# itshawi/data-accelerator

Hardware: AMD Instinct MI355X
Metric: events/sec (node) + p99 latency, SimulatedData IoT Flow (higher is better)
Workload: dtype fp64/int64 columns (no reduced precision)

## Files before the change

dxa/io/kafka_device.py:

```python
from __future__ import annotations

import ctypes
from dataclasses import dataclass
from typing import List, Optional, Sequence, Tuple

import numpy as np
import torch

_PLAN_ERRS = {-2: "message format is not v2", -3: "CRC mismatch", -5: "codec decoded on the host only",
              -7: "malformed compressed payload (LZ4 / snappy / zstd)", -8: "dependent-block LZ4 frame", -9: "offset deltas with gaps"}


TORCH_DT = {np.dtype(np.int32): torch.int32, np.dtype(np.int64): torch.int64, np.dtype(np.uint8): torch.uint8}


class Unsupported(Exception):
    """The fetch needs the host decoder."""


_BOUND = False


def _lib():
    global _BOUND
    from ..ops.serialize import lib
    L = lib()
    if not _BOUND:
        p, i64, i32 = ctypes.c_void_p, ctypes.c_int64, ctypes.c_int
        L.dxa_kafka_plan.argtypes = [p, i64, i64, i32, p, p] + [p] * 14
        L.dxa_kafka_plan.restype = ctypes.c_int
        _BOUND = True
    return L


@dataclass
class FetchPlan:
    b_count: np.ndarray
    b_base: np.ndarray
    b_skip: np.ndarray
    b_keep: np.ndarray
    b_first: np.ndarray
    b_nblk: np.ndarray
    b_rec0: np.ndarray
    k_comp_off: np.ndarray
    k_comp_len: np.ndarray
    k_stored: np.ndarray
    k_out_off: np.ndarray
    k_cap: np.ndarray
    out_bytes: int
    next_offset: int
    nbytes: int = 0
    packed: Optional[torch.Tensor] = None
    layout: Optional[list] = None
    b_crc_off: Optional[np.ndarray] = None
    b_crc_len: Optional[np.ndarray] = None
    b_crc: Optional[np.ndarray] = None

    def __post_init__(self):
        n = int(self.b_count.shape[0])
        for name, dt in (("b_crc_off", np.int64), ("b_crc_len", np.int32), ("b_crc", np.int32)):
            if getattr(self, name) is None:
                setattr(self, name, np.zeros(n, dt))

    @property
    def nbat(self) -> int:
        return int(self.b_count.shape[0])

    @property
    def nblk(self) -> int:
        return int(self.k_comp_off.shape[0])

    @property
    def nrec(self) -> int:
        return int(self.b_keep.sum()) if self.nbat else 0

    def last_offsets(self) -> np.ndarray:
        return self.b_base + self.b_skip + self.b_keep - 1


def plan_fetch(data, min_offset: int, verify_crc: bool = True) -> FetchPlan:
    a = np.frombuffer(data, dtype=np.uint8) if not isinstance(data, np.ndarray) else data
    L = _lib()
    counts = np.zeros(5, dtype=np.int64)
    nxt = ctypes.c_int64(0)
    rc = L.dxa_kafka_plan(a.ctypes.data, a.size, min_offset, int(verify_crc), counts.ctypes.data,
                          ctypes.byref(nxt), *([None] * 14))
    if rc:
        raise Unsupported(_PLAN_ERRS.get(rc, f"plan error {rc}"))
    nbat, nblk = int(counts[0]), int(counts[1])
    arr = dict(b_count=np.zeros(nbat, np.int32), b_base=np.zeros(nbat, np.int64),
               b_skip=np.zeros(nbat, np.int32), b_first=np.zeros(nbat, np.int32), b_nblk=np.zeros(nbat, np.int32),
               b_rec0=np.zeros(nbat, np.int64), k_comp_off=np.zeros(nblk, np.int64),
               k_comp_len=np.zeros(nblk, np.int32), k_stored=np.zeros(nblk, np.uint8),
               k_out_off=np.zeros(nblk, np.int64), k_cap=np.zeros(nblk, np.int64),
               b_crc_off=np.zeros(nbat, np.int64), b_crc_len=np.zeros(nbat, np.int32), b_crc=np.zeros(nbat, np.int32))
    order = ["b_count", "b_base", "b_skip", "b_first", "b_nblk", "b_rec0", "k_comp_off", "k_comp_len", "k_stored",
             "k_out_off", "k_cap", "b_crc_off", "b_crc_len", "b_crc"]
    rc = L.dxa_kafka_plan(a.ctypes.data, a.size, min_offset, int(verify_crc), counts.ctypes.data,
                          ctypes.byref(nxt), *[arr[k].ctypes.data for k in order])
    if rc:
        raise Unsupported(_PLAN_ERRS.get(rc, f"plan error {rc}"))
    keep = (arr["b_count"] - arr["b_skip"]).astype(np.int32)
    return FetchPlan(b_keep=keep, out_bytes=int(counts[3]), next_offset=nxt.value, nbytes=int(a.size), **arr)


_ARRAYS = [("b_count", np.int32, "b"), ("b_base", np.int64, "b"), ("b_skip", np.int32, "b"),
           ("b_keep", np.int32, "b"), ("b_first", np.int32, "b"), ("b_nblk", np.int32, "b"),
           ("b_rec0", np.int64, "b"), ("k_comp_off", np.int64, "k"), ("k_comp_len", np.int32, "k"),
           ("k_stored", np.uint8, "k"), ("k_out_off", np.int64, "k"), ("k_cap", np.int64, "k"),
           ("b_crc_off", np.int64, "b"), ("b_crc_len", np.int32, "b"), ("b_crc", np.int32, "b")]


class PlanBuffer:

    def __init__(self):
        self.buf: Optional[torch.Tensor] = None
        self.busy = None
        self.reserved = False

    def free(self) -> bool:
        return not self.reserved and (self.busy is None or self.busy.query())

    def release(self, event=None):
        self.busy = event
        self.reserved = False

    def carve(self, nbat: int, nblk: int):
        layout, pos = [], 0
        for name, dt, kind in _ARRAYS:
            cnt = nbat if kind == "b" else nblk
            layout.append((name, pos, cnt))
            pos += (cnt * np.dtype(dt).itemsize + 15) // 16 * 16
        if self.buf is None or self.buf.numel() < pos:
            self.buf = torch.empty(max(pos, 1) * 5 // 4 + 64, dtype=torch.uint8, pin_memory=torch.cuda.is_available())
        raw = self.buf.numpy()
        arrs = {name: raw[off:off + cnt * np.dtype(dt).itemsize].view(dt)
                for (name, off, cnt), (_, dt, _k) in zip(layout, _ARRAYS)}
        return arrs, layout, pos


class PlanBufferPool:

    def __init__(self):
        self.bufs: List[PlanBuffer] = []
        self._lock = __import__("threading").Lock()

    def get(self) -> PlanBuffer:
        with self._lock:
            for b in self.bufs:
                if b.free():
                    b.reserved = True
                    return b
            b = PlanBuffer()
            b.reserved = True
            self.bufs.append(b)
            return b


def plan_many(data: np.ndarray, bounds: Sequence[Tuple[int, int]], min_offsets: Sequence[int],
              threads: int = 16, buffer: Optional[PlanBuffer] = None, verify_crc: bool = True) -> FetchPlan:
    L = _lib()
    if not hasattr(L, "_plan_many_bound"):
        p, i64, i32 = ctypes.c_void_p, ctypes.c_int64, ctypes.c_int
        L.dxa_kafka_plan_count.argtypes = [p, i64, p, p, p, i32, i32, p, p]
        L.dxa_kafka_plan_fill.argtypes = [p, i64, p, p, p, i32, p] + [p] * 14
        L._plan_many_bound = True
    ns = len(bounds)
    so = np.array([b[0] for b in bounds], np.int64)
    sl = np.array([b[1] - b[0] for b in bounds], np.int64)
    mo = np.array(list(min_offsets), np.int64)
    counts = np.zeros((ns, 4), np.int64)
    nxt = np.zeros(ns, np.int64)
    rc = L.dxa_kafka_plan_count(data.ctypes.data, ns, so.ctypes.data, sl.ctypes.data, mo.ctypes.data,
                                int(verify_crc), threads,
                                counts.ctypes.data, nxt.ctypes.data)
    if rc:
        raise Unsupported(_PLAN_ERRS.get(rc, f"plan error {rc}"))
    nbat, nblk = int(counts[:, 0].sum()), int(counts[:, 1].sum())
    buffer = buffer or PlanBuffer()
    arrs, layout, used = buffer.carve(nbat, nblk)
    rc = L.dxa_kafka_plan_fill(data.ctypes.data, ns, so.ctypes.data, sl.ctypes.data, mo.ctypes.data, threads,
                               counts.ctypes.data, *[arrs[n].ctypes.data for n in
                                                     ("b_count", "b_base", "b_skip", "b_first", "b_nblk", "b_rec0",
                                                      "k_comp_off", "k_comp_len", "k_stored", "k_out_off",
                                                      "k_cap", "b_crc_off", "b_crc_len", "b_crc")])
    if rc:
        raise Unsupported(_PLAN_ERRS.get(rc, f"plan error {rc}"))
    np.subtract(arrs["b_count"], arrs["b_skip"], out=arrs["b_keep"])
    plan = FetchPlan(out_bytes=int(counts[:, 3].sum()), next_offset=int(nxt.max()) if ns else 0,
                     nbytes=int((so + sl).max()) if ns else 0, packed=buffer.buf[:used], layout=layout, **arrs)
    plan.buffer = buffer
    return plan


def merge(plans: Sequence[Tuple[FetchPlan, int]]) -> FetchPlan:
    if not plans:
        return FetchPlan(*(np.zeros(0, t) for t in (np.int32, np.int64, np.int32, np.int32, np.int32, np.int32,
                                                      np.int64, np.int64, np.int32, np.uint8, np.int64, np.int64)),
                         out_bytes=0, next_offset=0)
    cat = lambda k: np.concatenate([getattr(p, k) for p, _ in plans])
    blk0, out0, rec0 = [], [], []
    nb = ob = nr = 0
    for p, _ in plans:
        blk0.append(nb)
        out0.append(ob)
        rec0.append(nr)
        nb += p.nblk
        ob += p.out_bytes
        nr += p.nrec
    return FetchPlan(
        b_count=cat("b_count"), b_base=cat("b_base"), b_skip=cat("b_skip"), b_keep=cat("b_keep"),
        b_first=np.concatenate([p.b_first + b for (p, _), b in zip(plans, blk0)]).astype(np.int32),
        b_nblk=cat("b_nblk"),
        b_rec0=np.concatenate([_rec0(p) + r for (p, _), r in zip(plans, rec0)]),
        k_comp_off=np.concatenate([p.k_comp_off + at for p, at in plans]),
        k_comp_len=cat("k_comp_len"), k_stored=cat("k_stored"),
        k_out_off=np.concatenate([p.k_out_off + o for (p, _), o in zip(plans, out0)]),
        k_cap=cat("k_cap"), out_bytes=ob, next_offset=plans[-1][0].next_offset,
        nbytes=max(at + p.nbytes for p, at in plans),
        b_crc_off=np.concatenate([p.b_crc_off + at for p, at in plans]), b_crc_len=cat("b_crc_len"),
        b_crc=cat("b_crc"))


def _rec0(p: FetchPlan) -> np.ndarray:
    if not p.nbat:
        return np.zeros(0, np.int64)
    c = np.cumsum(p.b_keep, dtype=np.int64)
    return c - p.b_keep


def trim(p: FetchPlan, max_records: int) -> FetchPlan:
    if p.nrec <= max_records:
        return p
    keep = p.b_keep.copy()
    cum = np.cumsum(keep, dtype=np.int64)
    cut = int(np.searchsorted(cum, max_records, side="left"))
    before = int(cum[cut - 1]) if cut else 0
    keep[cut] = max_records - before
    keep[cut + 1:] = 0
    q = FetchPlan(**{**p.__dict__, "b_keep": keep.astype(np.int32)})
    q.b_rec0 = _rec0(q)
    q.next_offset = int(p.b_base[cut] + p.b_skip[cut] + keep[cut])
    return q


class DeviceRecordDecoder:

    def __init__(self, device, chunks: int = 4, copy_stream=None, decode_stream=None, track: bool = True,
                 verify_crc: bool = False):
        self.device = torch.device(device)
        self.verify_crc = verify_crc
        self.crc_stream = torch.cuda.Stream(self.device) if verify_crc else None
        self.chunks = max(1, chunks)
        cus = torch.cuda.get_device_properties(self.device).multi_processor_count
        self.min_blocks_per_chunk = cus * 64
        self.copy_stream = copy_stream or torch.cuda.Stream(self.device)
        self.decode_stream = decode_stream or torch.cuda.Stream(self.device)
        self.track = track
        self.checks: List["DecodeStatus"] = []

    def decode(self, staging: torch.Tensor, plan: FetchPlan):
        from ..engine.processor import RawBatch
        from ..ops import native as N
        dev = self.device
        n = plan.nrec
        if plan.packed is None:
            if not hasattr(self, "_packs"):
                self._packs = PlanBufferPool()
            pb = self._packs.get()
            plan.buffer = pb
            arrs, layout, used = pb.carve(plan.nbat, plan.nblk)
            for name, _dt, _k in _ARRAYS:
                arrs[name][...] = getattr(plan, name)
            packed = pb.buf[:used]
        else:
            packed, layout = plan.packed, plan.layout
        with torch.cuda.stream(self.copy_stream):
            dtab = packed.to(dev, non_blocking=True)
            ddata = torch.empty(plan.nbytes + 32, dtype=torch.uint8, device=dev)
            tab_ev = torch.cuda.Event()
            tab_ev.record(self.copy_stream)
        if getattr(plan, "buffer", None) is not None:
            plan.buffer.release(tab_ev)
        views = {name: dtab[off:off + cnt * np.dtype(dt).itemsize].view(TORCH_DT[np.dtype(dt)])
                 for (name, off, cnt), (_, dt, _k) in zip(layout, _ARRAYS)}
        tabs = [views[k] for k in ("k_comp_off", "k_comp_len", "k_stored", "k_out_off", "k_cap", "b_count",
                                   "b_skip", "b_keep", "b_first", "b_nblk", "b_rec0")]
        crc_tabs = [views[k] for k in ("b_crc_off", "b_crc_len", "b_crc")]
        co, cl, sd, oo, cap, bc, bs, bk, bf, bn, br = tabs
        with torch.cuda.stream(self.decode_stream):
            out = torch.empty(plan.out_bytes + 64, dtype=torch.uint8, device=dev)
            produced = torch.empty(max(1, plan.nblk), dtype=torch.int64, device=dev)
            bstat = torch.empty(max(1, plan.nblk), dtype=torch.int32, device=dev)
            offs = torch.empty(n + 1, dtype=torch.int64, device=dev)
            ends = torch.empty(max(1, n), dtype=torch.int64, device=dev)
            rstat = torch.empty(max(1, plan.nbat), dtype=torch.int32, device=dev)
        self.decode_stream.wait_event(tab_ev)
        st = self.decode_stream.cuda_stream
        nb = plan.nblk
        chunks = max(1, min(self.chunks, nb // max(1, self.min_blocks_per_chunk)))
        kinds = set(np.unique(plan.k_stored[:nb]).tolist()) if nb else set()
        has_gzip, has_snappy, has_zstd = 2 in kinds, 3 in kinds, 4 in kinds
        bounds = np.linspace(0, nb, chunks + 1).astype(np.int64)
        ev_last = tab_ev
        copied = 0
        for k in range(chunks):
            b0, b1 = int(bounds[k]), int(bounds[k + 1])
            if b1 <= b0:
                continue
            lo = copied
            hi = plan.nbytes if b1 == nb else int(plan.k_comp_off[b1])
            copied = hi
            N.call("dxa_memcpy_h2d_async", ddata.data_ptr() + lo, staging.data_ptr() + lo, hi - lo,
                   self.copy_stream.cuda_stream)
            ev = torch.cuda.Event()
            ev.record(self.copy_stream)
            ev_last = ev
            self.decode_stream.wait_event(ev)
            N.call("dxa_lz4_decode_into", N.ptr(ddata), N.ptr(co[b0:b1]), N.ptr(cl[b0:b1]), N.ptr(sd[b0:b1]),
                   N.ptr(oo[b0:b1]), N.ptr(cap[b0:b1]), b1 - b0, N.ptr(out), N.ptr(produced[b0:b1]),
                   N.ptr(bstat[b0:b1]), st)
            for present, entry in ((has_gzip, "dxa_inflate_into"), (has_snappy, "dxa_snappy_decode_into"),
                                   (has_zstd, "dxa_zstd_decode_into")):
                if present:
                    N.call(entry, N.ptr(ddata), N.ptr(co[b0:b1]), N.ptr(cl[b0:b1]), N.ptr(sd[b0:b1]),
                           N.ptr(oo[b0:b1]), N.ptr(cap[b0:b1]), b1 - b0, N.ptr(out), N.ptr(produced[b0:b1]),
                           N.ptr(bstat[b0:b1]), st)
        with torch.cuda.stream(self.decode_stream):
            offs[n:].fill_(plan.out_bytes)
        N.call("dxa_kafka_records", N.ptr(out), plan.nbat, N.ptr(bc), N.ptr(bs), N.ptr(bk), N.ptr(bf), N.ptr(bn),
               N.ptr(br), N.ptr(oo), N.ptr(cap), N.ptr(produced), N.ptr(bstat), N.ptr(offs), N.ptr(ends),
               N.ptr(rstat), st)
        done = torch.cuda.Event()
        done.record(self.decode_stream)
        if self.verify_crc:
            cs = self.crc_stream
            cs.wait_event(ev_last)
            with torch.cuda.stream(cs):
                cstat = torch.empty(max(1, plan.nbat), dtype=torch.int32, device=dev)
            N.call("dxa_kafka_crc", N.ptr(ddata), plan.nbat, *[N.ptr(t) for t in crc_tabs], N.ptr(cstat),
                   cs.cuda_stream)
            cs.wait_event(done)
            with torch.cuda.stream(cs):
                bad = (rstat[:plan.nbat] != 0).sum() + (cstat[:plan.nbat] != 0).sum()
                status = DecodeStatus(bad, cs)
            for t in (ddata, dtab, rstat):
                t.record_stream(cs)
        else:
            with torch.cuda.stream(self.decode_stream):
                status = DecodeStatus((rstat[:plan.nbat] != 0).sum(), self.decode_stream)
        for t in (ddata, produced, bstat, dtab):
            t.record_stream(self.decode_stream)
        if self.track:
            self.checks.append(status)
        self._inflight = [(e, b) for e, b in getattr(self, "_inflight", []) if not e.query()] + \
            [(status.event if self.verify_crc else done, (staging, packed))]
        return RawBatch(out, offs, n, ends=ends[:n], source_bytes=plan.nbytes, status=status), done

    def check(self):
        pending, self.checks = self.checks, []
        bad = sum(s.failed() for s in pending)
        if bad:
            raise DecodeError(f"{bad} Kafka record batch(es) failed to decode on the device")


class DecodeError(ValueError):
    pass


class DecodeStatus:

    __slots__ = ("host", "event")

    def __init__(self, bad: torch.Tensor, stream):
        self.host = torch.empty(1, dtype=torch.int64, pin_memory=True)
        self.host.copy_(bad.reshape(1), non_blocking=True)
        self.event = torch.cuda.Event()
        self.event.record(stream)

    def failed(self) -> int:
        self.event.synchronize()
        return int(self.host[0])

    def raise_if_failed(self, what: str = "batch"):
        bad = self.failed()
        if bad:
            raise DecodeError(f"{what}: {bad} Kafka record batch(es) failed to decode on the device")


_CRC_POLY = 0x82F63B78


def _multmodp(a: int, b: int) -> int:
    p = 0
    m = 1 << 31
    while m:
        if a & m:
            p ^= b
        b = (b >> 1) ^ _CRC_POLY if b & 1 else b >> 1
        m >>= 1
    return p


def _x2n_table():
    t, p = [], 1 << 30
    for _ in range(32):
        t.append(p)
        p = _multmodp(p, p)
    return t


_X2N = _x2n_table()


def _raw_crc(reg: int, data: bytes) -> int:
    for byte in data:
        reg ^= byte
        for _ in range(8):
            reg = (reg >> 1) ^ _CRC_POLY if reg & 1 else reg >> 1
    return reg


def _x8n(n: int) -> int:
    p, sq = 1 << 31, 1 << 30
    for _ in range(3):
        sq = _multmodp(sq, sq)
    while n:
        if n & 1:
            p = _multmodp(sq, p)
        sq = _multmodp(sq, sq)
        n >>= 1
    return p


def crc32c_segmented(data: bytes, base_align: int = 0) -> int:
    n = len(data)
    e = base_align + n
    E = e - (e & 7)
    if E - base_align < 8:
        return ~_raw_crc(0xFFFFFFFF, data) & 0xFFFFFFFF
    nrow = (E - base_align + 511) // 512
    r0 = E - nrow * 512
    msg = bytearray(data)
    for q in range(min(4, n)):
        msg[q] ^= 0xFF

    def byte_at(pos):
        q = pos - base_align
        return msg[q] if 0 <= q < n else 0
    total = 0
    for lane in range(64):
        acc = 0
        for r in range(nrow):
            a = r0 + r * 512 + lane * 8
            acc = _raw_crc(acc, bytes(byte_at(a + k) for k in range(8)))
            if r + 1 < nrow:
                acc = _multmodp(_x8n(504), acc)
        if acc:
            total ^= _multmodp(_x8n((63 - lane) * 8), acc)
    reg = _raw_crc(total, bytes(msg[E - base_align:]))
    return ~reg & 0xFFFFFFFF


def decode_on_host_like(staging: np.ndarray, plan: FetchPlan, verify_crc: bool = False):
    from ..ops import lz4
    out = np.zeros(plan.out_bytes + 64, dtype=np.uint8)
    starts, ends = [], []
    for i in range(plan.nbat):
        if verify_crc:
            lo = int(plan.b_crc_off[i])
            got = crc32c_segmented(staging[lo:lo + int(plan.b_crc_len[i])].tobytes(), lo & 7)
            if got != int(plan.b_crc[i]) & 0xFFFFFFFF:
                raise DecodeError(f"batch {i}: CRC-32C mismatch")
        f, nb = int(plan.b_first[i]), int(plan.b_nblk[i])
        p = int(plan.k_out_off[f])
        end = p
        for b in range(f, f + nb):
            src = staging[plan.k_comp_off[b]: plan.k_comp_off[b] + plan.k_comp_len[b]]
            kind = int(plan.k_stored[b])
            if kind == 2:
                import zlib
                raw = zlib.decompressobj(-15).decompress(src.tobytes())
            elif kind == 3:
                from .kafka import snappy_decompress
                raw = snappy_decompress(src.tobytes())
            elif kind == 4:
                from .kafka import zstd_decompress
                raw = zstd_decompress(src.tobytes())
            else:
                raw = src.tobytes() if kind else lz4.decompress_block(src.tobytes(), int(plan.k_cap[b]))
            out[end:end + len(raw)] = np.frombuffer(raw, np.uint8)
            end += len(raw)
        data = out

        def varint(p):
            u, s = 0, 0
            while True:
                c = int(data[p])
                p += 1
                u |= (c & 0x7F) << s
                s += 7
                if not c & 0x80:
                    return (u >> 1) ^ -(u & 1), p
        skip, keep, count = int(plan.b_skip[i]), int(plan.b_keep[i]), int(plan.b_count[i])
        for r in range(min(count, skip + keep)):
            ln, p = varint(p)
            rec_end = p + ln
            p += 1
            _, p = varint(p)
            _, p = varint(p)
            kl, p = varint(p)
            p += max(kl, 0)
            vl, p = varint(p)
            if r >= skip:
                starts.append(p)
                ends.append(p + max(vl, 0))
            p = rec_end
        assert p <= end
    return out, np.array(starts, np.int64), np.array(ends, np.int64)
```

dxa/ops/csrc/lz4.hip:

```cpp
#include "dxa_common.h"

namespace {

struct InWin {
  const uint8_t* base;
  uintptr_t wb;
  uint4 w;
  __device__ __forceinline__ uint32_t at(int64_t q) {
    const uintptr_t a = reinterpret_cast<uintptr_t>(base + q);
    const uintptr_t b = a & ~(uintptr_t)15;
    if (b != wb) {
      wb = b;
      w = *reinterpret_cast<const uint4*>(b);
    }
    return dxa::window_byte(w, (uint32_t)(a - b));
  }
};

struct OutBuf {
  uint8_t* p;
  int64_t len;
  int head;
  int nacc;
  uint64_t a0, a1;
  uintptr_t wb;
  uint4 w;

  __device__ __forceinline__ void init(uint8_t* dst) {
    p = dst; len = 0; nacc = 0; a0 = a1 = 0; wb = 0;
    head = (int)((16 - ((uintptr_t)dst & 15)) & 15);
  }
  __device__ __forceinline__ void put(uint32_t c) {
    if (len < head) {
      p[len] = (uint8_t)c;
      wb = 0;
    } else {
      if (nacc < 8) a0 |= (uint64_t)c << (8 * nacc);
      else a1 |= (uint64_t)c << (8 * (nacc - 8));
      if (++nacc == 16) {
        uint64_t* q = reinterpret_cast<uint64_t*>(p + len - 15);
        __builtin_nontemporal_store(a0, q);
        __builtin_nontemporal_store(a1, q + 1);
        a0 = a1 = 0;
        nacc = 0;
      }
    }
    ++len;
  }
  __device__ __forceinline__ uint32_t get(int64_t q) {
    const int64_t acc0 = len - nacc;
    if (q >= acc0 && len >= head) {
      const int k = (int)(q - acc0);
      return (uint32_t)(((k < 8) ? (a0 >> (8 * k)) : (a1 >> (8 * (k - 8)))) & 0xff);
    }
    const uintptr_t a = reinterpret_cast<uintptr_t>(p + q);
    const uintptr_t b = a & ~(uintptr_t)15;
    if (b != wb) {
      wb = b;
      asm volatile("" ::: "memory");
      w = *reinterpret_cast<const uint4*>(b);
    }
    return dxa::window_byte(w, (uint32_t)(a - b));
  }
  __device__ __forceinline__ void finish() {
    uint8_t* q = p + len - nacc;
    for (int k = 0; k < nacc; ++k) q[k] = (uint8_t)((k < 8 ? a0 >> (8 * k) : a1 >> (8 * (k - 8))) & 0xff);
  }
};

enum : int32_t { LZ_OK = 0, LZ_TRUNC = 1, LZ_OFFSET = 2, LZ_OVERFLOW = 3, LZ_SIZE = 4 };

template <bool WRITE>
__device__ int32_t run_block(const uint8_t* src, int64_t n, uint8_t* dst, int64_t cap, int64_t& produced) {
  InWin in{src, 0, make_uint4(0, 0, 0, 0)};
  OutBuf out;
  if (WRITE) out.init(dst);
  int64_t ip = 0, op = 0;
  while (ip < n) {
    const uint32_t token = in.at(ip++);
    int64_t lit = token >> 4;
    if (lit == 15) {
      uint32_t b;
      do { if (ip >= n) return LZ_TRUNC; b = in.at(ip++); lit += b; } while (b == 255);
    }
    if (lit > n - ip) return LZ_TRUNC;
    if (lit > cap - op) return LZ_OVERFLOW;
    if (WRITE) for (int64_t k = 0; k < lit; ++k) out.put(in.at(ip + k));
    ip += lit;
    op += lit;
    if (ip >= n) break;
    if (n - ip < 2) return LZ_TRUNC;
    const int64_t off = (int64_t)in.at(ip) | ((int64_t)in.at(ip + 1) << 8);
    ip += 2;
    if (off == 0 || off > op) return LZ_OFFSET;
    int64_t ml = token & 15;
    if (ml == 15) {
      uint32_t b;
      do { if (ip >= n) return LZ_TRUNC; b = in.at(ip++); ml += b; } while (b == 255);
    }
    ml += 4;
    if (ml > cap - op) return LZ_OVERFLOW;
    if (WRITE) {
      const int64_t s = op - off;
      if (off == 1) {
        const uint32_t c = out.get(s);
        for (int64_t k = 0; k < ml; ++k) out.put(c);
      } else {
        for (int64_t k = 0; k < ml; ++k) out.put(out.get(s + k));
      }
    }
    op += ml;
  }
  if (WRITE) out.finish();
  produced = op;
  return LZ_OK;
}

__global__ __launch_bounds__(256) void lz4_sizes_kernel(const uint8_t* __restrict__ src,
                                                        const int64_t* __restrict__ comp_off,
                                                        const int32_t* __restrict__ comp_len,
                                                        const uint8_t* __restrict__ stored, int64_t nb,
                                                        int64_t max_block, int64_t* __restrict__ out_len,
                                                        int32_t* __restrict__ status) {
  const int64_t b = (int64_t)blockIdx.x * blockDim.x + threadIdx.x;
  if (b >= nb) return;
  if (stored[b]) { out_len[b] = comp_len[b]; status[b] = LZ_OK; return; }
  int64_t produced = 0;
  const int32_t rc = run_block<false>(src + comp_off[b], comp_len[b], nullptr, max_block, produced);
  out_len[b] = rc == LZ_OK ? produced : 0;
  status[b] = rc;
}

constexpr int kWaitVm0 = 0xF70;

template <int G>
__global__ __launch_bounds__(256) void lz4_decode_group_kernel(const uint8_t* __restrict__ src,
                                                               const int64_t* __restrict__ comp_off,
                                                               const int32_t* __restrict__ comp_len,
                                                               const uint8_t* __restrict__ stored,
                                                               const int64_t* __restrict__ out_off,
                                                               const int64_t* __restrict__ out_len, int64_t nb,
                                                               uint8_t* __restrict__ dst,
                                                               int32_t* __restrict__ status,
                                                               int64_t* __restrict__ produced) {
  static_assert(G == 8 || G == 16, "group width");
  constexpr int NW = 16 / G, LPL = 16 / G, BPL = 32 / G, LOG_G = G == 8 ? 3 : 4;
  constexpr int WB = 64, PIPE = 32;
  const int64_t b = ((int64_t)blockIdx.x * 256 + threadIdx.x) / G;
  const int gl = (int)(threadIdx.x & (G - 1));
  const int gbase = (int)((threadIdx.x & 63) & ~(G - 1));
  if (b >= nb) return;
  const uint8_t kd = stored[b];
  if (kd > 1) return;
  const int32_t n = comp_len[b];
  const int64_t cap64 = out_len[b];
  const uint8_t* in = src + comp_off[b];
  uint8_t* out = dst + out_off[b];
  auto put = [&](bool on, int32_t pos, uint32_t v) {
    if (on) out[pos] = (uint8_t)v;
  };
  auto fetch = [&](bool on, int32_t pos) -> uint32_t { return on ? (uint32_t)out[pos] : 0u; };
  if (kd) {
    if (produced ? (n > cap64) : (n != cap64)) {
      if (gl == 0) status[b] = LZ_SIZE;
      return;
    }
    for (int32_t k = gl; k < n; k += G) out[k] = in[k];
    if (gl == 0) {
      status[b] = LZ_OK;
      if (produced) produced[b] = n;
    }
    return;
  }
  if (cap64 > INT32_MAX || cap64 < 0 || n < 0) {
    if (gl == 0) status[b] = LZ_OVERFLOW;
    return;
  }
  const int32_t cap = (int32_t)cap64;
  const int32_t shift = (int32_t)(reinterpret_cast<uintptr_t>(in) & 3);
  const uint8_t* a0 = in - shift;
  const int32_t lim = shift + n + 16;
  uint32_t X[NW];
  auto ld = [&](int32_t w0) {
#pragma unroll
    for (int k = 0; k < NW; ++k) {
      const int32_t q = w0 + 4 * (gl + G * k);
      X[k] = (q + 4 <= lim) ? *reinterpret_cast<const uint32_t*>(a0 + q) : 0u;
    }
    __builtin_amdgcn_s_waitcnt(kWaitVm0);
  };
  auto wbyte = [&](int32_t r) -> uint32_t {
    const int d = (r >> 2) & (G * NW - 1);
    const int addr = (gbase + (d & (G - 1))) << 2;
    uint32_t v = (uint32_t)__builtin_amdgcn_ds_bpermute(addr, (int)X[0]);
    if constexpr (NW == 2) {
      const uint32_t v1 = (uint32_t)__builtin_amdgcn_ds_bpermute(addr, (int)X[1]);
      v = (d >> LOG_G) ? v1 : v;
    }
    return (v >> ((r & 3) * 8)) & 0xffu;
  };
  int32_t xb = 0;
  ld(0);
  auto get = [&](int32_t p) -> uint32_t {
    if (p - xb >= WB) {
      xb = p & ~3;
      ld(xb);
    }
    return wbyte(p - xb);
  };
  const int32_t iend = shift + n;
  int32_t ip = shift, op = 0, rc = LZ_OK, done = 0;
  int32_t pdst = 0, pml = 0;
  uint32_t pv[BPL];
#pragma unroll
  for (int k = 0; k < BPL; ++k) pv[k] = 0;
  auto flush = [&]() {
#pragma unroll
    for (int k = 0; k < BPL; ++k) put(gl + G * k < pml, pdst + G * k + gl, pv[k]);
  };
  while (ip < iend) {
    if (ip - xb > WB - 16) {
      xb = ip & ~3;
      ld(xb);
    }
    const int32_t r = ip - xb;
    const uint32_t token = wbyte(r);
    int32_t lit = (int32_t)(token >> 4);
    const int32_t mlc = (int32_t)(token & 15);
    const bool has_ext = mlc == 15 && lit < 15 && r + lit + 4 <= WB;
    const uint32_t mext = has_ext ? wbyte(r + lit + 3) : 0u;
    const int32_t fml = mlc + 4 + (int32_t)mext;
    const int32_t fhdr = lit + 3 + (mlc == 15 ? 1 : 0);
    if (lit < 15 && (mlc < 15 || mext < 255) && r + fhdr <= WB && iend - ip >= fhdr && cap - op >= lit + fml) {
#pragma unroll
      for (int k = 0; k < LPL; ++k) {
        const uint32_t lv = wbyte(r + 1 + G * k + gl);
        put(gl + G * k < lit, op + G * k + gl, lv);
      }
      const int32_t off = (int32_t)(wbyte(r + 1 + lit) | (wbyte(r + 2 + lit) << 8));
      ip += fhdr;
      op += lit;
      if (off == 0 || off > op) { rc = LZ_OFFSET; break; }
      const int32_t ml = fml;
      const int32_t s0 = op - off;
      const int32_t src_end = s0 + (off < ml ? off : ml);
      if (pml > 0 && (src_end > pdst || ml > PIPE)) {
        flush();
        pml = 0;
      }
      if (src_end > done) {
        __builtin_amdgcn_s_waitcnt(kWaitVm0);
        asm volatile("" ::: "memory");
        done = pml > 0 ? pdst : op;
      }
      if (ml > PIPE) {
        if (off >= ml) {
          for (int32_t c = 0; c < ml; c += G)
            if (c + gl < ml) out[op + c + gl] = out[s0 + c + gl];
        } else {
          for (int32_t c = 0; c < ml; c += G) {
            const uint32_t i = (uint32_t)(c + gl);
            if ((int32_t)i < ml) out[op + i] = out[s0 + (int32_t)(i % (uint32_t)off)];
          }
        }
        op += ml;
        continue;
      }
      uint32_t v[BPL];
      if (off >= ml) {
#pragma unroll
        for (int k = 0; k < BPL; ++k) v[k] = fetch(gl + G * k < ml, s0 + G * k + gl);
      } else {
        const uint32_t o = (uint32_t)off;
#pragma unroll
        for (int k = 0; k < BPL; ++k) v[k] = fetch(gl + G * k < ml, s0 + (int32_t)((uint32_t)(gl + G * k) % o));
      }
      if (pml > 0) flush();
      pdst = op;
      pml = ml;
#pragma unroll
      for (int k = 0; k < BPL; ++k) pv[k] = v[k];
      op += ml;
      continue;
    }
    if (pml > 0) {
      flush();
      pml = 0;
    }
    ++ip;
    if (lit == 15) {
      uint32_t e;
      do {
        if (ip >= iend) { rc = LZ_TRUNC; break; }
        e = get(ip);
        ++ip;
        lit += (int32_t)e;
      } while (e == 255);
      if (rc != LZ_OK) break;
    }
    if (lit > iend - ip) { rc = LZ_TRUNC; break; }
    if (lit > cap - op) { rc = LZ_OVERFLOW; break; }
    for (int32_t c = 0; c < lit; c += G)
      if (c + gl < lit) out[op + c + gl] = a0[ip + c + gl];
    ip += lit;
    op += lit;
    if (ip >= iend) break;
    if (iend - ip < 2) { rc = LZ_TRUNC; break; }
    const int32_t off = (int32_t)(get(ip) | (get(ip + 1) << 8));
    ip += 2;
    if (off == 0 || off > op) { rc = LZ_OFFSET; break; }
    int32_t ml = mlc;
    if (ml == 15) {
      uint32_t e;
      do {
        if (ip >= iend) { rc = LZ_TRUNC; break; }
        e = get(ip);
        ++ip;
        ml += (int32_t)e;
      } while (e == 255);
      if (rc != LZ_OK) break;
    }
    ml += 4;
    if (ml > cap - op) { rc = LZ_OVERFLOW; break; }
    const int32_t s0 = op - off;
    if (s0 + (off < ml ? off : ml) > done) {
      __builtin_amdgcn_s_waitcnt(kWaitVm0);
      asm volatile("" ::: "memory");
      done = op;
    }
    if (off >= ml) {
      for (int32_t c = 0; c < ml; c += G)
        if (c + gl < ml) out[op + c + gl] = out[s0 + c + gl];
    } else {
      for (int32_t c = 0; c < ml; c += G) {
        const uint32_t i = (uint32_t)(c + gl);
        if ((int32_t)i < ml) out[op + i] = out[s0 + (int32_t)(i % (uint32_t)off)];
      }
    }
    op += ml;
  }
  if (pml > 0) flush();
  if (rc == LZ_OK && !produced && op != cap) rc = LZ_SIZE;
  if (gl == 0) {
    status[b] = rc;
    if (produced) produced[b] = op;
  }
}

}

DXA_API int dxa_lz4_block_sizes(const void* src, const void* comp_off, const void* comp_len, const void* stored,
                                int64_t nb, int64_t max_block, void* out_len, void* status, void* st) {
  if (nb <= 0) return 0;
  hipLaunchKernelGGL(lz4_sizes_kernel, dim3((unsigned)((nb + 255) / 256)), dim3(256), 0, (hipStream_t)st,
                     (const uint8_t*)src, (const int64_t*)comp_off, (const int32_t*)comp_len, (const uint8_t*)stored,
                     nb, max_block, (int64_t*)out_len, (int32_t*)status);
  return (int)hipGetLastError();
}

template <int G>
static int launch_group(int64_t nb, hipStream_t s, const uint8_t* src, const int64_t* co, const int32_t* cl,
                        const uint8_t* sd, const int64_t* oo, const int64_t* ol, uint8_t* dst, int32_t* status,
                        int64_t* produced) {
  const dim3 grid((unsigned)((nb * G + 255) / 256));
  hipLaunchKernelGGL((lz4_decode_group_kernel<G>), grid, dim3(256), 0, s, src, co, cl, sd, oo, ol, nb, dst, status,
                     produced);
  return (int)hipGetLastError();
}

DXA_API int dxa_lz4_decode(const void* src, const void* comp_off, const void* comp_len, const void* stored,
                           const void* out_off, const void* out_len, int64_t nb, int64_t max_out, void* dst,
                           void* status, void* st) {
  if (nb <= 0) return 0;
  const hipStream_t s = (hipStream_t)st;
  return launch_group<16>(nb, s, (const uint8_t*)src, (const int64_t*)comp_off, (const int32_t*)comp_len,
                          (const uint8_t*)stored, (const int64_t*)out_off, (const int64_t*)out_len, (uint8_t*)dst,
                          (int32_t*)status, (int64_t*)nullptr);
}

DXA_API int dxa_lz4_decode_into(const void* src, const void* comp_off, const void* comp_len, const void* stored,
                                const void* out_off, const void* cap, int64_t nb, void* dst, void* produced,
                                void* status, void* st) {
  if (nb <= 0) return 0;
  const hipStream_t s = (hipStream_t)st;
  const uint8_t* s8 = (const uint8_t*)src;
  const int64_t* co = (const int64_t*)comp_off;
  const int32_t* cl = (const int32_t*)comp_len;
  const uint8_t* sd = (const uint8_t*)stored;
  const int64_t* oo = (const int64_t*)out_off;
  const int64_t* cp = (const int64_t*)cap;
  return launch_group<16>(nb, s, s8, co, cl, sd, oo, cp, (uint8_t*)dst, (int32_t*)status, (int64_t*)produced);
}

DXA_API int dxa_memcpy_h2d_async(void* dst, const void* src, int64_t n, void* st) {
  if (n <= 0) return 0;
  return (int)hipMemcpyAsync(dst, src, (size_t)n, hipMemcpyHostToDevice, (hipStream_t)st);
}
```

Before: 252.2 million.

## Decode up to sixteen LZ4 sequences per lane group in parallel

Reworks the LZ4 group decoder so each 16-lane group speculatively parses sequence headers inside a 128-byte input window. It chains token positions through bpermute, prefix-sums output offsets with DPP, and copies literals and matches for many short sequences at once using wide unaligned stores. The goal is to remove the serial one-sequence-at-a-time loop that dominates small-record decoding. It also pins waves per EU, drops the G template, and lowers the minimum blocks per chunk so batches get split into more chunks. The cost is much more complex dependency handling between overlapping matches, with risk of correctness bugs and extra register pressure.

```diff
diff --git a/dxa/io/kafka_device.py b/dxa/io/kafka_device.py
--- a/dxa/io/kafka_device.py
+++ b/dxa/io/kafka_device.py
@@ -253,7 +253,7 @@
         self.crc_stream = torch.cuda.Stream(self.device) if verify_crc else None
         self.chunks = max(1, chunks)
         cus = torch.cuda.get_device_properties(self.device).multi_processor_count
-        self.min_blocks_per_chunk = cus * 64
+        self.min_blocks_per_chunk = cus * 16
         self.copy_stream = copy_stream or torch.cuda.Stream(self.device)
         self.decode_stream = decode_stream or torch.cuda.Stream(self.device)
         self.track = track
diff --git a/dxa/ops/csrc/lz4.hip b/dxa/ops/csrc/lz4.hip
--- a/dxa/ops/csrc/lz4.hip
+++ b/dxa/ops/csrc/lz4.hip
@@ -132,20 +132,23 @@
 }
 
 constexpr int kWaitVm0 = 0xF70;
-
-template <int G>
-__global__ __launch_bounds__(256) void lz4_decode_group_kernel(const uint8_t* __restrict__ src,
-                                                               const int64_t* __restrict__ comp_off,
-                                                               const int32_t* __restrict__ comp_len,
-                                                               const uint8_t* __restrict__ stored,
-                                                               const int64_t* __restrict__ out_off,
-                                                               const int64_t* __restrict__ out_len, int64_t nb,
-                                                               uint8_t* __restrict__ dst,
-                                                               int32_t* __restrict__ status,
-                                                               int64_t* __restrict__ produced) {
-  static_assert(G == 8 || G == 16, "group width");
-  constexpr int NW = 16 / G, LPL = 16 / G, BPL = 32 / G, LOG_G = G == 8 ? 3 : 4;
-  constexpr int WB = 64, PIPE = 32;
+typedef uint32_t __attribute__((aligned(1), may_alias)) u32_unaligned;
+struct __attribute__((packed, may_alias)) U8 { uint32_t a, b; };
+struct __attribute__((packed, may_alias)) U16 { uint32_t a, b, c, d; };
+
+__device__ __forceinline__ int32_t row_scan16(int32_t x) {
+  x += __builtin_amdgcn_update_dpp(0, x, 0x111, 0xf, 0xf, false);
+  x += __builtin_amdgcn_update_dpp(0, x, 0x112, 0xf, 0xf, false);
+  x += __builtin_amdgcn_update_dpp(0, x, 0x114, 0xf, 0xf, false);
+  x += __builtin_amdgcn_update_dpp(0, x, 0x118, 0xf, 0xf, false);
+  return x;
+}
+
+__global__ __launch_bounds__(256) __attribute__((amdgpu_waves_per_eu(8, 8))) void lz4_decode_group_kernel(
+    const uint8_t* __restrict__ src, const int64_t* __restrict__ comp_off, const int32_t* __restrict__ comp_len,
+    const uint8_t* __restrict__ stored, const int64_t* __restrict__ out_off, const int64_t* __restrict__ out_len,
+    int64_t nb, uint8_t* __restrict__ dst, int32_t* __restrict__ status, int64_t* __restrict__ produced) {
+  constexpr int G = 16, WB = 128;
   const int64_t b = ((int64_t)blockIdx.x * 256 + threadIdx.x) / G;
   const int gl = (int)(threadIdx.x & (G - 1));
   const int gbase = (int)((threadIdx.x & 63) & ~(G - 1));
@@ -156,10 +159,6 @@
   const int64_t cap64 = out_len[b];
   const uint8_t* in = src + comp_off[b];
   uint8_t* out = dst + out_off[b];
-  auto put = [&](bool on, int32_t pos, uint32_t v) {
-    if (on) out[pos] = (uint8_t)v;
-  };
-  auto fetch = [&](bool on, int32_t pos) -> uint32_t { return on ? (uint32_t)out[pos] : 0u; };
   if (kd) {
     if (produced ? (n > cap64) : (n != cap64)) {
       if (gl == 0) status[b] = LZ_SIZE;
@@ -180,27 +179,33 @@
   const int32_t shift = (int32_t)(reinterpret_cast<uintptr_t>(in) & 3);
   const uint8_t* a0 = in - shift;
   const int32_t lim = shift + n + 16;
-  uint32_t X[NW];
+  uint32_t X0, X1;
   auto ld = [&](int32_t w0) {
-#pragma unroll
-    for (int k = 0; k < NW; ++k) {
-      const int32_t q = w0 + 4 * (gl + G * k);
-      X[k] = (q + 4 <= lim) ? *reinterpret_cast<const uint32_t*>(a0 + q) : 0u;
-    }
+    const int32_t q = w0 + 4 * gl;
+    X0 = (q + 4 <= lim) ? *reinterpret_cast<const uint32_t*>(a0 + q) : 0u;
+    X1 = (q + 68 <= lim) ? *reinterpret_cast<const uint32_t*>(a0 + q + 64) : 0u;
     __builtin_amdgcn_s_waitcnt(kWaitVm0);
+    asm volatile("" ::: "memory");
   };
-  auto wbyte = [&](int32_t r) -> uint32_t {
-    const int d = (r >> 2) & (G * NW - 1);
+  auto wdw = [&](int32_t d) -> uint32_t {
     const int addr = (gbase + (d & (G - 1))) << 2;
-    uint32_t v = (uint32_t)__builtin_amdgcn_ds_bpermute(addr, (int)X[0]);
-    if constexpr (NW == 2) {
-      const uint32_t v1 = (uint32_t)__builtin_amdgcn_ds_bpermute(addr, (int)X[1]);
-      v = (d >> LOG_G) ? v1 : v;
-    }
-    return (v >> ((r & 3) * 8)) & 0xffu;
+    const uint32_t v0 = (uint32_t)__builtin_amdgcn_ds_bpermute(addr, (int)X0);
+    const uint32_t v1 = (uint32_t)__builtin_amdgcn_ds_bpermute(addr, (int)X1);
+    return (d & G) ? v1 : v0;
+  };
+  auto wbyte = [&](int32_t r) -> uint32_t { return (wdw(r >> 2) >> ((r & 3) * 8)) & 0xffu; };
+  auto wdword = [&](int32_t r) -> uint32_t {
+    const uint32_t lo = wdw(r >> 2), hi = wdw((r >> 2) + 1);
+    return (uint32_t)((((uint64_t)hi << 32) | lo) >> ((r & 3) * 8));
+  };
+  auto w8 = [&](int32_t r, uint32_t& lo, uint32_t& hi) {
+    const uint32_t d0 = wdw(r >> 2), d1 = wdw((r >> 2) + 1), d2 = wdw((r >> 2) + 2);
+    const int sh = (r & 3) * 8;
+    lo = (uint32_t)((((uint64_t)d1 << 32) | d0) >> sh);
+    hi = (uint32_t)((((uint64_t)d2 << 32) | d1) >> sh);
   };
   int32_t xb = 0;
-  ld(0);
+  X0 = X1 = 0;
   auto get = [&](int32_t p) -> uint32_t {
     if (p - xb >= WB) {
       xb = p & ~3;
@@ -210,83 +215,144 @@
   };
   const int32_t iend = shift + n;
   int32_t ip = shift, op = 0, rc = LZ_OK, done = 0;
-  int32_t pdst = 0, pml = 0;
-  uint32_t pv[BPL];
+  while (ip < iend) {
+    xb = ip & ~3;
+    ld(xb);
+    done = op;
+    const int32_t r0 = ip - xb;
+    uint32_t jw0 = 0, jw1 = 0;
 #pragma unroll
-  for (int k = 0; k < BPL; ++k) pv[k] = 0;
-  auto flush = [&]() {
-#pragma unroll
-    for (int k = 0; k < BPL; ++k) put(gl + G * k < pml, pdst + G * k + gl, pv[k]);
-  };
-  while (ip < iend) {
-    if (ip - xb > WB - 16) {
-      xb = ip & ~3;
-      ld(xb);
-    }
-    const int32_t r = ip - xb;
-    const uint32_t token = wbyte(r);
+    for (int m = 0; m < 4; ++m) {
+      const uint32_t b0 = (X0 >> (8 * m)) & 0xffu, b1 = (X1 >> (8 * m)) & 0xffu;
+      const int32_t l0 = (int32_t)(b0 >> 4), l1 = (int32_t)(b1 >> 4);
+      const int32_t e0 = 4 * gl + m + l0 + 3 + ((b0 & 15u) == 15u ? 1 : 0);
+      const int32_t e1 = 64 + 4 * gl + m + l1 + 3 + ((b1 & 15u) == 15u ? 1 : 0);
+      jw0 |= ((l0 < 15) ? (uint32_t)e0 : 255u) << (8 * m);
+      jw1 |= (((l1 < 15) & (e1 <= WB)) ? (uint32_t)e1 : 255u) << (8 * m);
+    }
+    int32_t pos = r0, mypos = gl == 0 ? r0 : 255;
+    for (int j = 1; j < G; ++j) {
+      if (__builtin_amdgcn_ballot_w64(pos < WB) == 0) break;
+      const int addr = (gbase + ((pos >> 2) & (G - 1))) << 2;
+      const uint32_t w0 = (uint32_t)__builtin_amdgcn_ds_bpermute(addr, (int)jw0);
+      const uint32_t w1 = (uint32_t)__builtin_amdgcn_ds_bpermute(addr, (int)jw1);
+      const int32_t nx = (int32_t)((((pos & 64) ? w1 : w0) >> ((pos & 3) * 8)) & 0xffu);
+      pos = pos < WB ? nx : pos;
+      mypos = gl == j ? pos : mypos;
+    }
+    const bool has = mypos < WB;
+    const int32_t mp = has ? mypos : 0;
+    const uint32_t qtok = wbyte(mp);
+    const int32_t qlit = (int32_t)(qtok >> 4);
+    const int32_t qmlc = (int32_t)(qtok & 15);
+    const uint32_t dw = wdword(mp + 1 + qlit);
+    const int32_t mext = qmlc == 15 ? (int32_t)((dw >> 16) & 0xffu) : 0;
+    const int32_t qml = qmlc + 4 + mext;
+    const int32_t qhdr = qlit + 3 + (qmlc == 15 ? 1 : 0);
+    const int32_t qoff = (int32_t)(dw & 0xffffu);
+    const int32_t myip = xb + mp;
+    bool plain = has & (qlit < 15) & (mext < 255) & (mp + qhdr <= WB) & (iend - myip >= qhdr) & (qoff >= qml);
+    const int32_t adv = plain ? qlit + qml : 0;
+    const int32_t myop = op + row_scan16(adv) - adv;
+    plain = plain & (cap - myop >= qlit + qml) & (qoff <= myop + qlit);
+    const uint32_t okb = (uint32_t)(__builtin_amdgcn_ballot_w64(plain) >> gbase) & 0xffffu;
+    const int32_t cnt = __builtin_ctz(~okb | 0x10000u);
+    const int32_t my_dst = myop + qlit;
+    const uint32_t my_om = (uint32_t)qoff | ((uint32_t)qml << 16);
+    if (cnt > 0) {
+      const int last = (gbase + cnt - 1) << 2;
+      ip = __builtin_amdgcn_ds_bpermute(last, myip + qhdr);
+      op = __builtin_amdgcn_ds_bpermute(last, my_dst + qml);
+      const bool act = gl < cnt;
+      uint8_t* lq = out + myop;
+      const bool l8 = act & (qlit >= 8), l4 = act & (qlit >= 4) & (qlit < 8), l1 = act & (qlit >= 1) & (qlit < 4);
+      const int32_t lt = qlit - (qlit >= 8 ? 8 : 4);
+      uint32_t x0, x1, y0, y1;
+      w8(mp + 1, x0, x1);
+      w8(mp + 1 + (lt > 0 ? lt : 0), y0, y1);
+      if (l8) {
+        *reinterpret_cast<U8*>(lq) = U8{x0, x1};
+        *reinterpret_cast<U8*>(lq + lt) = U8{y0, y1};
+      }
+      if (l4) {
+        *reinterpret_cast<u32_unaligned*>(lq) = x0;
+        *reinterpret_cast<u32_unaligned*>(lq + lt) = y0;
+      }
+      if (l1) {
+        lq[0] = (uint8_t)x0;
+        lq[qlit >> 1] = (uint8_t)(x0 >> (8 * (qlit >> 1)));
+        lq[qlit - 1] = (uint8_t)(x0 >> (8 * (qlit - 1)));
+      }
+    }
+    if (cnt > 0) {
+      bool pend = gl < cnt;
+      const int32_t mlen = (int32_t)(my_om >> 16);
+      uint8_t* md = out + my_dst;
+      const uint8_t* ms = md - (int32_t)(my_om & 0xffffu);
+      const int32_t send = my_dst - (int32_t)(my_om & 0xffffu) + mlen;
+      for (;;) {
+        const uint64_t pb = __builtin_amdgcn_ballot_w64(pend);
+        if (pb == 0) break;
+        const uint32_t gb = (uint32_t)(pb >> gbase) & 0xffffu;
+        const int first = gb ? __builtin_ctz(gb) : 0;
+        const int32_t F = __builtin_amdgcn_ds_bpermute((gbase + first) << 2, my_dst);
+        const bool ready = pend && send <= F;
+        if (__builtin_amdgcn_ballot_w64(ready && send > done) != 0) {
+          __builtin_amdgcn_s_waitcnt(kWaitVm0);
+          asm volatile("" ::: "memory");
+          if (gb) done = F;
+        }
+        const bool c4 = ready & (mlen < 8), c8 = ready & (mlen >= 8) & (mlen < 16), c16 = ready & (mlen >= 16);
+        const int32_t t = mlen - (mlen >= 16 ? 16 : mlen >= 8 ? 8 : 4);
+        const int32_t t1 = t < 16 ? t : 16, t2 = t > 16 ? t - 16 : 0;
+        U16 e0 = {}, e1 = {}, e2 = {}, e3 = {};
+        if (c4) {
+          e0.a = *reinterpret_cast<const u32_unaligned*>(ms);
+          e1.a = *reinterpret_cast<const u32_unaligned*>(ms + t);
+        }
+        if (c8) {
+          const U8 b0 = *reinterpret_cast<const U8*>(ms), b1 = *reinterpret_cast<const U8*>(ms + t);
+          e0.a = b0.a, e0.b = b0.b, e1.a = b1.a, e1.b = b1.b;
+        }
+        if (c16) {
+          e0 = *reinterpret_cast<const U16*>(ms);
+          e1 = *reinterpret_cast<const U16*>(ms + t);
+        }
+        const bool c32 = c16 & (mlen > 32);
+        if (c32) {
+          e2 = *reinterpret_cast<const U16*>(ms + t1);
+          e3 = *reinterpret_cast<const U16*>(ms + t2);
+        }
+        if (c4) {
+          *reinterpret_cast<u32_unaligned*>(md) = e0.a;
+          *reinterpret_cast<u32_unaligned*>(md + t) = e1.a;
+        }
+        if (c8) {
+          *reinterpret_cast<U8*>(md) = U8{e0.a, e0.b};
+          *reinterpret_cast<U8*>(md + t) = U8{e1.a, e1.b};
+        }
+        if (c16) {
+          *reinterpret_cast<U16*>(md) = e0;
+          *reinterpret_cast<U16*>(md + t) = e1;
+        }
+        if (c32) {
+          *reinterpret_cast<U16*>(md + t1) = e2;
+          *reinterpret_cast<U16*>(md + t2) = e3;
+          for (int32_t k = 32; k < t2; k += 32) {
+            const int32_t k1 = k + 16 < t2 ? k + 16 : t2;
+            e0 = *reinterpret_cast<const U16*>(ms + k);
+            e1 = *reinterpret_cast<const U16*>(ms + k1);
+            *reinterpret_cast<U16*>(md + k) = e0;
+            *reinterpret_cast<U16*>(md + k1) = e1;
+          }
+        }
+        pend = pend && !ready;
+      }
+      continue;
+    }
+    const uint32_t token = get(ip);
     int32_t lit = (int32_t)(token >> 4);
     const int32_t mlc = (int32_t)(token & 15);
-    const bool has_ext = mlc == 15 && lit < 15 && r + lit + 4 <= WB;
-    const uint32_t mext = has_ext ? wbyte(r + lit + 3) : 0u;
-    const int32_t fml = mlc + 4 + (int32_t)mext;
-    const int32_t fhdr = lit + 3 + (mlc == 15 ? 1 : 0);
-    if (lit < 15 && (mlc < 15 || mext < 255) && r + fhdr <= WB && iend - ip >= fhdr && cap - op >= lit + fml) {
-#pragma unroll
-      for (int k = 0; k < LPL; ++k) {
-        const uint32_t lv = wbyte(r + 1 + G * k + gl);
-        put(gl + G * k < lit, op + G * k + gl, lv);
-      }
-      const int32_t off = (int32_t)(wbyte(r + 1 + lit) | (wbyte(r + 2 + lit) << 8));
-      ip += fhdr;
-      op += lit;
-      if (off == 0 || off > op) { rc = LZ_OFFSET; break; }
-      const int32_t ml = fml;
-      const int32_t s0 = op - off;
-      const int32_t src_end = s0 + (off < ml ? off : ml);
-      if (pml > 0 && (src_end > pdst || ml > PIPE)) {
-        flush();
-        pml = 0;
-      }
-      if (src_end > done) {
-        __builtin_amdgcn_s_waitcnt(kWaitVm0);
-        asm volatile("" ::: "memory");
-        done = pml > 0 ? pdst : op;
-      }
-      if (ml > PIPE) {
-        if (off >= ml) {
-          for (int32_t c = 0; c < ml; c += G)
-            if (c + gl < ml) out[op + c + gl] = out[s0 + c + gl];
-        } else {
-          for (int32_t c = 0; c < ml; c += G) {
-            const uint32_t i = (uint32_t)(c + gl);
-            if ((int32_t)i < ml) out[op + i] = out[s0 + (int32_t)(i % (uint32_t)off)];
-          }
-        }
-        op += ml;
-        continue;
-      }
-      uint32_t v[BPL];
-      if (off >= ml) {
-#pragma unroll
-        for (int k = 0; k < BPL; ++k) v[k] = fetch(gl + G * k < ml, s0 + G * k + gl);
-      } else {
-        const uint32_t o = (uint32_t)off;
-#pragma unroll
-        for (int k = 0; k < BPL; ++k) v[k] = fetch(gl + G * k < ml, s0 + (int32_t)((uint32_t)(gl + G * k) % o));
-      }
-      if (pml > 0) flush();
-      pdst = op;
-      pml = ml;
-#pragma unroll
-      for (int k = 0; k < BPL; ++k) pv[k] = v[k];
-      op += ml;
-      continue;
-    }
-    if (pml > 0) {
-      flush();
-      pml = 0;
-    }
     ++ip;
     if (lit == 15) {
       uint32_t e;
@@ -339,7 +405,6 @@
     }
     op += ml;
   }
-  if (pml > 0) flush();
   if (rc == LZ_OK && !produced && op != cap) rc = LZ_SIZE;
   if (gl == 0) {
     status[b] = rc;
@@ -358,12 +423,11 @@
   return (int)hipGetLastError();
 }
 
-template <int G>
 static int launch_group(int64_t nb, hipStream_t s, const uint8_t* src, const int64_t* co, const int32_t* cl,
                         const uint8_t* sd, const int64_t* oo, const int64_t* ol, uint8_t* dst, int32_t* status,
                         int64_t* produced) {
-  const dim3 grid((unsigned)((nb * G + 255) / 256));
-  hipLaunchKernelGGL((lz4_decode_group_kernel<G>), grid, dim3(256), 0, s, src, co, cl, sd, oo, ol, nb, dst, status,
+  const dim3 grid((unsigned)((nb * 16 + 255) / 256));
+  hipLaunchKernelGGL(lz4_decode_group_kernel, grid, dim3(256), 0, s, src, co, cl, sd, oo, ol, nb, dst, status,
                      produced);
   return (int)hipGetLastError();
 }
@@ -373,7 +437,7 @@
                            void* status, void* st) {
   if (nb <= 0) return 0;
   const hipStream_t s = (hipStream_t)st;
-  return launch_group<16>(nb, s, (const uint8_t*)src, (const int64_t*)comp_off, (const int32_t*)comp_len,
+  return launch_group(nb, s, (const uint8_t*)src, (const int64_t*)comp_off, (const int32_t*)comp_len,
                           (const uint8_t*)stored, (const int64_t*)out_off, (const int64_t*)out_len, (uint8_t*)dst,
                           (int32_t*)status, (int64_t*)nullptr);
 }
@@ -389,7 +453,7 @@
   const uint8_t* sd = (const uint8_t*)stored;
   const int64_t* oo = (const int64_t*)out_off;
   const int64_t* cp = (const int64_t*)cap;
-  return launch_group<16>(nb, s, s8, co, cl, sd, oo, cp, (uint8_t*)dst, (int32_t*)status, (int64_t*)produced);
+  return launch_group(nb, s, s8, co, cl, sd, oo, cp, (uint8_t*)dst, (int32_t*)status, (int64_t*)produced);
 }
 
 DXA_API int dxa_memcpy_h2d_async(void* dst, const void* src, int64_t n, void* st) {
```

Result: no change. 250.7 million (-0.6%).
